# allenai/embodied-clip

Measured on AMD Instinct MI355X. Metric: env-frames/sec (CLIP encode + policy fwd/bwd + PPO update), higher is better.
Workload: dtype bf16

## Files before the change

embodied_clip_amd/_lib.py:

```python
from __future__ import annotations

import ctypes as C
import os

_HERE = os.path.dirname(os.path.abspath(__file__))
LIB_PATH = os.environ.get("EC_AMD_LIB") or os.path.join(_HERE, "lib", "libec_amd.so")

c_void_p, c_int, c_size_t, c_float = C.c_void_p, C.c_int, C.c_size_t, C.c_float

SIGNATURES = {
    "ec_version": (c_int, []),
    "ec_strerror": (C.c_char_p, [c_int]),
    "ec_bind_streams": (c_int, [c_void_p, c_int, c_int]),
    "ec_stream_pair_overlap": (c_int, [c_void_p, c_void_p, c_int, c_void_p]),
    "ec_conv_bf16": (c_int, [c_void_p] * 5 + [c_int] * 8 + [c_void_p]),
    "ec_conv_bf16_ld": (c_int, [c_void_p] * 5 + [c_int] * 9 + [c_void_p]),
    "ec_conv3x3_img_pack": (c_int, [c_void_p, c_void_p, c_int, c_void_p]),
    "ec_conv3x3_img_bf16": (c_int, [c_void_p] * 4 + [c_int] * 5 + [c_void_p]),
    "ec_conv3x3_img_bf16_ld": (c_int, [c_void_p] * 4 + [c_int] * 6 + [c_void_p]),
    "ec_bneck3_packed_elems": (c_size_t, [c_int]),
    "ec_bneck3_pack_weights": (c_int, [c_void_p] * 4 + [c_int, c_void_p]),
    "ec_bneck_conv123_bf16": (c_int, [c_void_p] * 6 + [c_int] * 4 + [c_void_p]),
    "ec_bneck_packed_elems": (c_size_t, [c_int]),
    "ec_bneck_pack_weights": (c_int, [c_void_p] * 3 + [c_int, c_void_p]),
# ... 28 lines not shown
    "ec_rn50_workspace_bytes": (c_size_t, [c_void_p, c_int]),
    "ec_rn50_out_channels": (c_int, [c_void_p]),
    "ec_rn50_out_spatial": (c_int, [c_void_p]),
    "ec_rn50_forward": (c_int, [c_void_p, c_void_p, c_int, c_void_p, c_size_t, c_void_p, c_int, c_void_p]),
    "ec_stem_conv1_depth": (c_int, [c_void_p, c_float, c_float, c_void_p, c_void_p, c_void_p] + [c_int] * 4 + [c_void_p]),
    "ec_rn50_forward_depth": (c_int, [c_void_p, c_void_p, c_float, c_float, c_void_p, c_int, c_void_p, c_size_t, c_void_p, c_int,
                                      c_void_p]),
    "ec_spatial_mean_pair_bf16": (c_int, [c_void_p] * 3 + [c_int] * 3 + [c_void_p]),
    "ec_rn50_rgbd_workspace_bytes": (c_size_t, [c_void_p, c_int]),
    "ec_rn50_embed_rgbd": (c_int, [c_void_p, c_void_p, c_int, C.POINTER(c_float), C.POINTER(c_float), c_void_p, c_float, c_float,
                                   c_void_p, c_int, c_void_p, c_size_t, c_void_p, c_int, c_void_p]),
    "ec_rn50_num_ops": (c_int, [c_void_p]),
    "ec_rn50_plan_hash": (C.c_uint64, [c_void_p]),
    "ec_rn50_set_conv8_min_tiles": (c_int, [c_void_p, c_int]),
    "ec_rn50_set_l1_rebuild": (c_int, [c_void_p, c_int]),
    "ec_text_create": (c_int, [C.POINTER(c_void_p), c_int, c_int, c_int, c_int, c_int, c_int, c_void_p, c_size_t, c_void_p,
                               c_size_t]),
    "ec_text_destroy": (None, [c_void_p]),
    "ec_text_workspace_bytes": (c_size_t, [c_void_p, c_int]),
    "ec_text_forward": (c_int, [c_void_p, c_void_p, c_int, c_void_p, c_size_t, c_void_p, c_void_p]),
    "ec_probe_head": (c_int, [c_int, c_void_p, c_void_p, c_void_p, c_int, c_int, c_int, c_void_p, c_void_p, c_void_p,
                              c_void_p, c_void_p]),
    "ec_probe_pool3": (c_int, [c_void_p, c_void_p, c_int, c_int, c_int, c_int, c_void_p]),
    "ec_conv1x1_pair_pool_bf16": (c_int, [c_void_p] * 9 + [c_int] * 6 + [c_void_p]),
    "ec_conv1x1_pair_bf16": (c_int, [c_void_p] * 11 + [C.c_long, c_int, c_int, c_int, c_void_p]),
    "ec_conv1x1_pair_rebuild_bf16": (c_int, [c_void_p] * 13 + [C.c_long, c_int, c_int, c_int, c_void_p]),
    "ec_stem_conv1_u8": (c_int, [c_void_p, C.POINTER(c_float), C.POINTER(c_float), c_void_p, c_void_p, c_void_p]
                         + [c_int] * 4 + [c_void_p]),
    "ec_rn50_forward_u8": (c_int, [c_void_p, c_void_p, C.POINTER(c_float), C.POINTER(c_float), c_int, c_void_p,
                                   c_size_t, c_void_p, c_int, c_void_p]),
    "ec_gemm_f32": (c_int, [c_void_p] * 3 + [c_int] * 3 + [C.c_long] * 4 + [c_int, c_int] + [c_void_p] * 3 + [c_int]
                    + [c_void_p] * 2 + [c_int, c_void_p]),
    "ec_policy_create": (c_int, [C.POINTER(c_void_p), c_void_p]),
    "ec_policy_destroy": (None, [c_void_p]),
    "ec_policy_num_param_tensors": (c_int, [c_void_p]),
    "ec_policy_flat_size": (c_size_t, [c_void_p]),
    "ec_policy_param_offset": (c_int, [c_void_p, c_int, C.POINTER(c_size_t), C.POINTER(c_size_t)]),
    "ec_policy_workspace_bytes": (c_size_t, [c_void_p, c_int, c_int, c_int]),
    "ec_policy_forward": (c_int, [c_void_p, c_void_p, c_void_p, c_int, c_void_p, c_void_p, c_void_p, c_int, c_int,
                                  c_void_p, c_size_t, c_int, c_void_p, c_void_p, c_void_p]),
    "ec_policy_forward2": (c_int, [c_void_p, c_void_p, c_void_p, c_void_p, c_int, c_void_p, c_void_p, c_void_p, c_int, c_int,
# ... 207 lines not shown
```

embodied_clip_amd/csrc/rn50.hip:

```cpp
#include <stdlib.h>

#include <new>
#include <vector>

#include "common.h"


namespace {

enum OpKind { OP_STEM1, OP_CONV, OP_POOL, OP_PAIR, OP_BNECK, OP_STEM7, OP_BTAIL, OP_CAT, OP_CONV_POOLOUT };

constexpr int BUF_NONE = -1, BUF_IN = -2, BUF_OUT = -3;

struct Slot { size_t w = 0, b = 0; };

struct Conv {
    int src, dst, res;
    int H, W, Cin, Cout, ks, pool, act;
    int stride;
    Slot at;
    int ldo = 0, ocol = 0;
    int img_max = 0;
    size_t wimg_off = 0;
};

// ... 17 lines not shown

}

struct ec_rn50 {
    int width, res, out_c, out_sp;
    int tv = 0;
    std::vector<Op> ops;
    size_t max_elems_per_frame;
    const float* stem_w;
    const uint16_t* w;
    const float* bias;
    size_t n_w, n_b;
    int conv8_min_tiles = 0;
    int layers4[4] = {0, 0, 0, 0};
    int l1_rebuild = 0;
    uint16_t* wbneck = nullptr;
    float* bias_cat = nullptr;
    ~ec_rn50() {
        if (wbneck) (void)hipFree(wbneck);
        if (bias_cat) (void)hipFree(bias_cat);
    }
};

namespace {
constexpr int NBUF = 5;
inline size_t align_up(size_t v, size_t a) { return (v + a - 1) / a * a; }

enum TowerKind { CLIP = 0, TV_BOTTLENECK = 1, TV_BASIC = 2 };

struct Blk {
    int li, planes, inplanes, stride;
    int R, Ro;
    int x, out;
    int y;
    bool ds, last_of_layer;
    Slot c1, c2, c3, dsc;
};
struct Arch {
    TowerKind kind; int width, R1;
    bool l1_rebuild;
    Slot stem[3], total; std::vector<Blk> B;
};

Arch walk_arch(TowerKind kind, int width, int sc, const int* layers4, int R, bool l1_rebuild = false) {
    Arch a{kind, width, R, l1_rebuild};
    Slot& at = a.total;
    auto take = [&](size_t Cout, size_t K) { const Slot s = at; at.w += Cout * K; at.b += Cout; return s; };
    a.stem[0] = take(kind == CLIP ? sc : width, 0);
    if (kind == CLIP) { a.stem[1] = take(sc, (size_t)9 * sc); a.stem[2] = take(width, (size_t)9 * sc); }
    const int expansion = kind == TV_BASIC ? 1 : 4;
    int inplanes = width, x = 0;
    for (int li = 0; li < 4; ++li)
        for (int b = 0; b < layers4[li]; ++b) {
            Blk k{li, width << li, inplanes, (b == 0 && li > 0) ? 2 : 1};
            const size_t p = k.planes, in = inplanes;
            k.ds = k.stride > 1 || inplanes != k.planes * expansion;
            k.last_of_layer = b + 1 == layers4[li];
            k.R = R; k.Ro = R / k.stride;
            k.x = x; k.y = k.out = (x == 0) ? 4 : 0;
            k.c1 = take(p, kind == TV_BASIC ? 9 * in : in);
// ... 203 lines not shown
                           : ec_bneck_pack_weights(h->w + o.c2.at.w, h->w + o.c3.at.w, h->wbneck + o.wpack_off, o.c2.Cin, nullptr);
        else if (o.kind == OP_CONV && o.c.img_max) rc = ec_conv3x3_img_pack(h->w + o.c.at.w, h->wbneck + o.c.wimg_off, o.c.Cin, nullptr);
        if (rc != EC_OK) return EC_ERR_LAUNCH;
    }
    (void)hipStreamSynchronize(nullptr);
    return EC_OK;
}

int stem_channels(int width) { return (width / 2 + 31) / 32 * 32; }

size_t plan_tower(std::vector<Op>& ops, const Arch& a, int res) {
    ops.clear();
    Plan p{ops};
    const int width = a.width, sc = stem_channels(width);
    const int x0 = a.B.empty() ? BUF_OUT : a.B[0].x;
    if (a.kind == CLIP) {
        const int R = res / 2;
        p.push(Op{OP_STEM1, mk_conv(BUF_IN, 1, BUF_NONE, res, res, 3, sc, 3, 0, EC_ACT_RELU, a.stem[0])}, R, R, sc);
        p.conv(mk_conv(1, 2, BUF_NONE, R, R, sc, sc, 3, 0, EC_ACT_RELU, a.stem[1]));
        p.conv(mk_conv(2, x0, BUF_NONE, R, R, sc, width, 3, 1, EC_ACT_RELU, a.stem[2]));
    } else {
        p.push(Op{OP_STEM7, mk_conv(BUF_IN, x0, BUF_NONE, res, res, 3, width, 7, 0, EC_ACT_RELU, a.stem[0])}, a.R1, a.R1, width);
    }
    Given g;
    for (size_t i = 0; i < a.B.size(); ++i)
        if (a.kind == TV_BASIC) plan_basic(p, a.B[i]);
        else g = plan_bottleneck(p, a, i, g);
    return p.mx;
}

bool l1_rebuild_ok(const Arch& a) {
    return a.kind == CLIP && a.B.size() >= 3 && a.B[0].ds && block_form(a, 0) == F_PAIR1 && block_form(a, 1) == F_PAIR1;
}

int rn50_build(ec_rn50_t** out, TowerKind kind, int width, const int* layers4, int input_resolution, const void* stem_w,
               const void* w_bf16, size_t n_w, const float* bias, size_t n_bias) {
    if (!out || !layers4 || !stem_w || !w_bf16 || !bias) return EC_ERR_ARG;
    if (width % 32 != 0 || width < 32 || input_resolution % 32 != 0) return EC_ERR_SHAPE;
    if (kind == TV_BASIC && (input_resolution < 32 || layers4[0] < 1 || layers4[1] < 1 || layers4[2] < 1 || layers4[3] < 1)) return EC_ERR_SHAPE;
    const int res = input_resolution;
    const Arch a = walk_arch(kind, width, stem_channels(width), layers4, res / 4);
    if (n_w != a.total.w || n_bias != a.total.b) return EC_ERR_SHAPE;
    ec_rn50* h = new (std::nothrow) ec_rn50();
    if (!h) return EC_ERR_ALLOC;
    h->width = width; h->res = res; h->tv = kind;
    std::copy(layers4, layers4 + 4, h->layers4);
    h->stem_w = (const float*)stem_w; h->w = (const uint16_t*)w_bf16; h->bias = bias;
// ... 25 lines not shown

extern "C" void ec_rn50_destroy(ec_rn50_t* h) { delete h; }
extern "C" int ec_rn50_out_channels(const ec_rn50_t* h) { return h ? h->out_c : 0; }
extern "C" int ec_rn50_out_spatial(const ec_rn50_t* h) { return h ? h->out_sp : 0; }
extern "C" int ec_rn50_num_ops(const ec_rn50_t* h) { return h ? (int)h->ops.size() : 0; }

extern "C" uint64_t ec_rn50_plan_hash(const ec_rn50_t* h) {
    if (!h) return 0;
    uint64_t x = 1469598103934665603ull;
    auto mix = [&](long v) {
        for (int i = 0; i < 8; ++i) { x ^= (uint64_t)((v >> (8 * i)) & 0xff); x *= 1099511628211ull; }
    };
    mix(ec_version()); mix((long)ec_config_hash());
    mix(h->width); mix(h->res); mix(h->conv8_min_tiles); mix(h->tv);
    if (h->l1_rebuild) mix(h->l1_rebuild);
    for (const Op& o : h->ops) {
        const Conv& c = o.kind == OP_PAIR || o.kind == OP_BNECK ? o.c3 : o.kind == OP_BTAIL ? o.c2 : o.c;
        long f[24] = {o.kind, c.src, c.dst, c.res, c.H, c.W, c.Cin, c.Cout, c.ks, c.pool, c.act, c.stride, -1, -1, 0, -1, 0, c.ldo, c.ocol, 0, -1, 0, 0, 0};
        if (o.kind == OP_POOL) {
            const long p[12] = {OP_POOL, o.pl.src, o.pl.dst, -1, o.pl.H, o.pl.W, o.pl.C, o.pl.C, 0, 0, 0, 1};
            std::copy(p, p + 12, f);
            f[17] = o.pl.ldo; f[18] = o.pl.ocol; f[23] = o.pl.pool_of;
        }
        if (o.kind == OP_PAIR) { f[12] = o.fold_ds ? o.ds.src : -1; f[13] = o.next_c1.dst; f[14] = o.next_c1.Cout; f[15] = o.pooled_dst; }
        if (o.kind == OP_BNECK) { f[1] = o.c2.src; f[8] = 3; f[16] = o.fold_c1; }
        if (o.kind == OP_BTAIL) { f[3] = -1; f[6] = o.cat.Ka + o.cat.Kb; f[12] = o.ds.src; f[14] = o.cat.Ka; f[19] = 1; }
        if (o.kind == OP_CAT) { f[0] = OP_CONV; f[14] = o.cat.Ka; f[19] = 1; }
        if (o.kind == OP_CONV_POOLOUT) { f[0] = OP_CONV; f[20] = o.pd.dst; f[21] = o.pd.ld; f[22] = o.pd.col; }
        for (long v : f) mix(v);
    }
    return x;
}

extern "C" int ec_rn50_set_conv8_min_tiles(ec_rn50_t* h, int n) {
    if (!h) return EC_ERR_ARG;
    h->conv8_min_tiles = n > 0 ? n : 0;
    return EC_OK;
}

extern "C" int ec_rn50_set_l1_rebuild(ec_rn50_t* h, int on) {
    if (!h) return EC_ERR_ARG;
    const Arch a = walk_arch((TowerKind)h->tv, h->width, stem_channels(h->width), h->layers4, h->res / 4, on != 0);
    if (!l1_rebuild_ok(a)) return EC_ERR_UNSUPPORTED;
    if ((on != 0) == (h->l1_rebuild != 0)) return EC_OK;
    std::vector<Op> ops;
    const size_t mx = plan_tower(ops, a, h->res);
    size_t tot = 0, btot = 0;
    plan_offsets(ops, tot, btot);
    if (mx != h->max_elems_per_frame) return EC_ERR_UNSUPPORTED;
    h->ops.swap(ops);
    h->l1_rebuild = on != 0;
    return EC_OK;
}

extern "C" size_t ec_rn50_workspace_bytes(const ec_rn50_t* h, int batch) {
    if (!h || batch <= 0) return 0;
    return NBUF * align_up(h->max_elems_per_frame * 2 * (size_t)batch, 256);
}

namespace {
struct FrameIn {
    enum Kind { F32, U8, DEPTH, RGBD } kind;
    const void* p;
    const float *mean3, *std3;
    float scale, shift;
    const float* stem_w9;
    const float* depth = nullptr;
// ... 77 lines not shown
        return ec_conv1x1_pair_rebuild_bf16(r.buf(c3.src), h->w + c3.at.w, h->bias + c3.at.b, r.buf(o.id_c3.src), h->w + o.id_c3.at.w,
                                            h->bias + o.id_c3.at.b, r.buf(o.id_ds.src), h->w + o.id_ds.at.w, h->bias + o.id_ds.at.b,
                                            r.buf(c3.dst), h->w + c1.at.w, h->bias + c1.at.b, r.buf(c1.dst), (long)r.nb * c3.H * c3.W,
                                            c3.Cin, c3.Cout, c1.Cout, r.stream);
    int rc = ec_conv1x1_pair_bf16(r.buf(c3.src), h->w + c3.at.w, h->bias + c3.at.b, o.fold_ds ? r.buf(o.ds.src) : nullptr,
                                  o.fold_ds ? h->w + o.ds.at.w : nullptr, o.fold_ds ? h->bias + o.ds.at.b : nullptr, r.opt(c3.res),
                                  o.no_y ? nullptr : r.buf(c3.dst), h->w + c1.at.w, h->bias + c1.at.b, r.buf(c1.dst), (long)r.nb * c3.H * c3.W, c3.Cin, c3.Cout,
                                  c1.Cout, r.stream);
    if (rc == EC_ERR_SHAPE && !o.fold_ds) {
        rc = run_conv(r, c3);
        if (rc == EC_OK) rc = run_conv(r, c1);
    }
    return rc;
}

bool bneck_fused(int nb) { return nb >= ec_config().rn50_bneck; }

int run_bneck(const Run& r, const Op& o) {
    const ec_rn50* h = r.h;
    const Conv &c1 = o.c1, &c2 = o.c2, &c3 = o.c3;
    if (bneck_fused(r.nb) && o.fold_c1)
        return ec_bneck_conv123_bf16(r.buf(c3.res), h->wbneck + o.wpack_off, h->bias + c1.at.b, h->bias + c2.at.b, h->bias + c3.at.b,
                                     r.buf(c3.dst), r.nb, c3.H, c3.W, c2.Cin, r.stream);
    if (bneck_fused(r.nb))
        return ec_bneck_conv23_bf16(r.buf(c2.src), h->wbneck + o.wpack_off, h->bias + c2.at.b, h->bias + c3.at.b, r.buf(c3.res),
                                    r.buf(c3.dst), r.nb, c3.H, c3.W, c2.Cin, r.stream);
    int rc = o.fold_c1 ? run_conv(r, c1) : EC_OK;
    if (rc == EC_OK) rc = run_conv(r, c2);
    return rc == EC_OK ? run_conv(r, c3) : rc;
}
// ... 30 lines not shown
    const size_t frame_bytes = (size_t)h->res * h->res * (in.kind == FrameIn::DEPTH ? 1 : 3) * (in.u8() ? 1 : 4);
    const size_t out_stride = (size_t)h->out_sp * h->out_sp * h->out_c;
    const hipStream_t stream = (hipStream_t)stream_main;
    auto pass = [&](Run r) -> int {
        for (const Op& o : h->ops) {
            int rc;
            switch (o.kind) {
                case OP_STEM1:
                case OP_STEM7: rc = run_stem(r, o); break;
                case OP_POOL: rc = run_pool(r, o); break;
                case OP_PAIR: rc = run_pair(r, o); break;
                case OP_BNECK: rc = run_bneck(r, o); break;
                case OP_BTAIL: rc = run_btail(r, o); break;
                case OP_CAT: rc = run_cat(r, o); break;
                case OP_CONV_POOLOUT: rc = run_conv_poolout(r, o); break;
                default: rc = run_conv(r, o.c);
            }
            if (rc != EC_OK) return rc;
        }
        return EC_OK;
    };
    unsigned char* const base = (unsigned char*)workspace;
    for (int b0 = 0; b0 < batch; b0 += chunk) {
        const int nb = std::min(chunk, batch - b0);
        const void* frames = (const unsigned char*)in.p + (size_t)b0 * frame_bytes;
        int rc;
        if (!rgbd) {
            const bool d = in.kind == FrameIn::DEPTH;
            rc = pass(Run{h, in, d ? nullptr : frames, d ? (const float*)frames : nullptr, nb, base, bufsz,
                          (uint16_t*)feat + (size_t)b0 * out_stride, stream, false});
// ... 52 lines not shown
```

embodied_clip_amd/encoder.py:

```python
from __future__ import annotations

import ctypes as C
from typing import Dict, List, Optional, Tuple

import torch

from . import _lib

BN_EPS = 1e-5


def _fold(w: torch.Tensor, sd: Dict[str, torch.Tensor], bn: str) -> Tuple[torch.Tensor, torch.Tensor]:
    g, b = sd[bn + ".weight"].float(), sd[bn + ".bias"].float()
    mu, var = sd[bn + ".running_mean"].float(), sd[bn + ".running_var"].float()
    s = g / torch.sqrt(var + BN_EPS)
    return w.float() * s.view(-1, 1, 1, 1), b - mu * s


def _layers(sd) -> List[int]:
    out = []
    for li in range(1, 5):
        n = 0
        while f"layer{li}.{n}.conv1.weight" in sd:
            n += 1
# ... 133 lines not shown
                self.h = None
        except Exception:
            pass

    def plan_hash(self) -> str:
        return f"{self.lib.ec_rn50_plan_hash(self.h):016x}"

    def set_conv8_min_tiles(self, n: int) -> None:
        _lib.check(self.lib.ec_rn50_set_conv8_min_tiles(self.h, int(n)), "ec_rn50_set_conv8_min_tiles")

    def set_l1_rebuild(self, on: bool = True) -> bool:
        rc = self.lib.ec_rn50_set_l1_rebuild(self.h, int(bool(on)))
        if rc == -6:
            return False
        _lib.check(rc, "ec_rn50_set_l1_rebuild")
        return True

    def _workspace(self, n: int) -> torch.Tensor:
        need = self.lib.ec_rn50_workspace_bytes(self.h, n)
        if self._ws is None or self._ws.numel() < need:
            self._ws = torch.empty(need, dtype=torch.uint8, device=self.device)
        return self._ws

    @_lib.on_device
    def forward(self, rgb: torch.Tensor, out: Optional[torch.Tensor] = None) -> torch.Tensor:
        assert rgb.is_cuda and rgb.dtype == torch.float32 and rgb.is_contiguous()
        B, R, R2, c3 = rgb.shape
        assert R == self.input_resolution and R2 == R and c3 == 3, rgb.shape
        S, Cc = self.out_spatial, self.out_channels
        if out is None:
# ... 478 lines not shown


@_guard_first
def conv1x1_pair_rebuild_bf16(a, w3, b3, i0, wi0, bi0, i1, wi1, bi1, w2, b2):
    lib = _lib.load()
    M, K0 = a.shape
    N, N2 = w3.shape[0], w2.shape[0]
    y = torch.empty((M, N), dtype=torch.bfloat16, device=a.device)
    z = torch.empty((M, N2), dtype=torch.bfloat16, device=a.device)
    _lib.check(lib.ec_conv1x1_pair_rebuild_bf16(a.data_ptr(), w3.data_ptr(), b3.data_ptr(), i0.data_ptr(), wi0.data_ptr(), bi0.data_ptr(),
                                                i1.data_ptr(), wi1.data_ptr(), bi1.data_ptr(), y.data_ptr(), w2.data_ptr(), b2.data_ptr(),
                                                z.data_ptr(), M, K0, N, N2, _lib.stream_ptr()), "ec_conv1x1_pair_rebuild_bf16")
    return y, z


def pack_text(sd: Dict[str, torch.Tensor]):
    sd = {k: v.detach().cpu().float() for k, v in sd.items()}
    vocab, D = sd["token_embedding.weight"].shape
    ctx = sd["positional_embedding"].shape[0]
    E = sd["text_projection"].shape[1]
    n = 0
    while f"transformer.resblocks.{n}.ln_1.weight" in sd:
        n += 1
    ws, fs = [], [sd["token_embedding.weight"].reshape(-1), sd["positional_embedding"].reshape(-1)]
    for i in range(n):
        p = f"transformer.resblocks.{i}."
        ws += [sd[p + "attn.in_proj_weight"], sd[p + "attn.out_proj.weight"], sd[p + "mlp.c_fc.weight"],
               sd[p + "mlp.c_proj.weight"]]
        fs += [sd[p + "ln_1.weight"], sd[p + "ln_1.bias"], sd[p + "attn.in_proj_bias"], sd[p + "attn.out_proj.bias"],
               sd[p + "ln_2.weight"], sd[p + "ln_2.bias"], sd[p + "mlp.c_fc.bias"], sd[p + "mlp.c_proj.bias"]]
# ... 63 lines not shown
```

embodied_clip_amd/engine.py:

```python
from __future__ import annotations

from collections import OrderedDict
from typing import Dict, List, Optional

import os
import random

import torch

from . import _lib
from . import synthetic as syn
from .dist import (allreduce_flat, check_job_seed, collective_active, gather_actor_counts, global_minibatch_sizes,
                   minibatch_bounds)
from .episodes import EpisodeTracker, NavEpisodeTracker, nav_env_tensors
from .encoder import AttentionPool, ClipTextEncoder, ImageNetBasicTrunk, ImageNetRN50Trunk, RN50Trunk, ViTEmbedder
from .policy import PolicyHandle
from .imitation import imitation_loss_raw, imitation_scratch
from .ppo import PPO_NARROW_MAX_A, FlatAdam, linear_decay_lr, ppo_loss_raw, ppo_wide_scratch

IMAGENET_ENCODERS = {
    "imagenet_rn18": ((2, 2, 2, 2), "basic", ImageNetBasicTrunk),
    "imagenet_rn34": ((3, 4, 6, 3), "basic", ImageNetBasicTrunk),
    "imagenet_rn50": ((3, 4, 6, 3), "bottleneck", ImageNetRN50Trunk),
}
# ... 340 lines not shown
            if frames_host:
                fshape = (n,) + tuple(self.env.frames.shape[2:])
                sl.stage = [torch.empty(fshape, dtype=self.env.frames.dtype, device=d) for _ in range(2)]
                sl.copy_stream = copy_streams[i]
                sl.copied = [torch.cuda.Event() for _ in range(2)]
                sl.consumed = [None, None]
                sl.k = 0
            self.slices.append(sl)
        self.encode_frames = n
        self._conv8_min_tiles = (50 if n >= 128 else (75 if n >= 64 else 0)) if ns == 2 else 0
        for e in encs:
            e.set_conv8_min_tiles(self._conv8_min_tiles)
        if encoder == "rn50":
            for e in encs:
                e.set_l1_rebuild(True)
        fused = os.environ.get("EC_ACT_FUSED_SAMPLE", "1") != "0"
        self._act_fused = fused and self.A + 1 <= 8
        self._act_wide = fused and 8 < self.A + 1 <= 257 and self.H <= 3576
        self.trunk_events: List = []
        self.time_trunk = False

    @property
    def feat(self) -> torch.Tensor:
        return self.slices[0].feat if self.ns == 1 else torch.cat([sl.feat for sl in self.slices], dim=1)

    @property
    def feat2(self) -> Optional[torch.Tensor]:
        if not self.dual:
            return None
        return self.slices[0].feat2 if self.ns == 1 else torch.cat([sl.feat2 for sl in self.slices], dim=1)
# ... 576 lines not shown
```

include/ec_amd.h:

```cpp
#ifndef EC_AMD_H
#define EC_AMD_H

#include <stddef.h>
#include <stdint.h>

#ifdef __cplusplus
extern "C" {
#endif

typedef void* ec_stream_t;
typedef void* ec_event_t;

enum {
    EC_OK = 0,
    EC_ERR_ARG = -1,
    EC_ERR_SHAPE = -2,
    EC_ERR_LAUNCH = -3,
    EC_ERR_WORKSPACE = -4,
    EC_ERR_ALLOC = -5,
    EC_ERR_UNSUPPORTED = -6
};

enum { EC_ACT_NONE = 0, EC_ACT_RELU = 1, EC_ACT_QUICKGELU = 2 };

// ... 41 lines not shown

int ec_stem_conv1(const float* rgb_nhwc, const float* w, const float* bias, void* out,
                  int B, int H, int W, int Cout, ec_stream_t stream);

int ec_stem_conv1_depth(const float* depth, float scale, float shift, const float* w9, const float* bias, void* out,
                        int B, int H, int W, int Cout, ec_stream_t stream);

int ec_conv1x1_pair_bf16(const void* a0, const void* w0, const float* b0, const void* a1, const void* w1,
                         const float* b1, const void* res, void* y, const void* w2, const float* b2, void* z,
                         long M, int K0, int N, int N2, ec_stream_t stream);

int ec_conv1x1_pair_rebuild_bf16(const void* a, const void* w3, const float* b3, const void* i0, const void* wi0,
                                 const float* bi0, const void* i1, const void* wi1, const float* bi1, void* y,
                                 const void* w2, const float* b2, void* z, long M, int K0, int N, int N2,
                                 ec_stream_t stream);

int ec_conv1x1_pair_pool_bf16(const void* a0, const void* w0, const float* b0, const void* res, void* y,
                              void* y_pooled, const void* w2, const float* b2, void* z, int B, int H, int W, int K0,
                              int N, int N2, ec_stream_t stream);

int ec_stem_conv1_u8(const uint8_t* rgb_u8_nhwc, const float* h_mean3, const float* h_std3, const float* w,
                     const float* bias, void* out, int B, int H, int W, int Cout, ec_stream_t stream);

size_t ec_bneck_packed_elems(int C);
int ec_bneck_pack_weights(const void* w2, const void* w3, void* packed, int C, ec_stream_t stream);
int ec_bneck_conv23_bf16(const void* c1, const void* packed, const float* b2, const float* b3,
                         const void* x, void* y, int B, int H, int W, int C, ec_stream_t stream);

size_t ec_bneck3_packed_elems(int C);
int ec_bneck3_pack_weights(const void* w1, const void* w2, const void* w3, void* packed, int C, ec_stream_t stream);
// ... 39 lines not shown
int ec_rn50_forward(const ec_rn50_t* h, const float* rgb_nhwc, int batch, void* workspace, size_t ws_bytes,
                    void* feat_bf16_nhwc, int chunk, ec_stream_t stream);
int ec_rn50_forward_u8(const ec_rn50_t* h, const uint8_t* rgb_u8_nhwc, const float* h_mean3, const float* h_std3,
                       int batch, void* workspace, size_t ws_bytes, void* feat_bf16_nhwc, int chunk,
                       ec_stream_t stream);
int ec_rn50_forward_depth(const ec_rn50_t* h, const float* depth, float scale, float shift, const float* stem_w9, int batch,
                          void* workspace, size_t ws_bytes, void* feat_bf16_nhwc, int chunk, ec_stream_t stream);
size_t ec_rn50_rgbd_workspace_bytes(const ec_rn50_t* h, int pairs);
int ec_rn50_embed_rgbd(const ec_rn50_t* h, const void* rgb, int rgb_u8, const float* h_mean3, const float* h_std3,
                       const float* depth, float scale, float shift, const float* stem_w9, int pairs, void* workspace,
                       size_t ws_bytes, float* embed, int chunk, ec_stream_t stream);
int ec_rn50_num_ops(const ec_rn50_t* h);
uint64_t ec_rn50_plan_hash(const ec_rn50_t* h);
int ec_rn50_set_conv8_min_tiles(ec_rn50_t* h, int n);
int ec_rn50_set_l1_rebuild(ec_rn50_t* h, int on);


enum {
    EC_GEMM_A_BF16 = 1,
    EC_GEMM_B_BF16 = 2,
    EC_GEMM_RELU = 4,
    EC_GEMM_ACCUMULATE = 8,
    EC_GEMM_SPLIT_PARTS = 16,
    EC_GEMM_3PRODUCTS = 32
};
int ec_gemm_f32(const void* A, const void* B, float* C, int M, int N, int K, long sam, long sak, long sbk, long sbn,
                int ldc, int flags, const float* bias, const float* gbias, const int* gidx, int group,
                const float* dmask, const float* rowscale, int splitk, ec_stream_t stream);

typedef struct {
// ... 231 lines not shown
```

Measured before the change: 63750.

## Fuse CLIP stem conv3 with avgpool and layer1 first 1x1 conv

Adds a new kernel that computes the third 3x3 stem conv with ReLU and 2x2 average pooling, then immediately applies the first bottleneck's 1x1 conv on the pooled tile while it is still in LDS. Both the pooled activation and the c1 output are written. A new plan op and setter wire it into the RN50 tower, and the engine enables it by default for rn50. The goal is to avoid one kernel launch and one round-trip through global memory for the pooled stem output. The cost is a specialized kernel tied to fixed channel counts (32 in, 64/64 out) that falls back to the old path for other shapes.

```diff
diff --git a/embodied_clip_amd/_lib.py b/embodied_clip_amd/_lib.py
--- a/embodied_clip_amd/_lib.py
+++ b/embodied_clip_amd/_lib.py
@@ -66,6 +66,7 @@
     "ec_rn50_plan_hash": (C.c_uint64, [c_void_p]),
     "ec_rn50_set_conv8_min_tiles": (c_int, [c_void_p, c_int]),
     "ec_rn50_set_l1_rebuild": (c_int, [c_void_p, c_int]),
+    "ec_rn50_set_stem_chain": (c_int, [c_void_p, c_int]),
     "ec_text_create": (c_int, [C.POINTER(c_void_p), c_int, c_int, c_int, c_int, c_int, c_int, c_void_p, c_size_t, c_void_p,
                                c_size_t]),
     "ec_text_destroy": (None, [c_void_p]),
@@ -77,6 +78,7 @@
     "ec_conv1x1_pair_pool_bf16": (c_int, [c_void_p] * 9 + [c_int] * 6 + [c_void_p]),
     "ec_conv1x1_pair_bf16": (c_int, [c_void_p] * 11 + [C.c_long, c_int, c_int, c_int, c_void_p]),
     "ec_conv1x1_pair_rebuild_bf16": (c_int, [c_void_p] * 13 + [C.c_long, c_int, c_int, c_int, c_void_p]),
+    "ec_stem3_pool_conv1_bf16": (c_int, [c_void_p] * 7 + [c_int] * 6 + [c_void_p]),
     "ec_stem_conv1_u8": (c_int, [c_void_p, C.POINTER(c_float), C.POINTER(c_float), c_void_p, c_void_p, c_void_p]
                          + [c_int] * 4 + [c_void_p]),
     "ec_rn50_forward_u8": (c_int, [c_void_p, c_void_p, C.POINTER(c_float), C.POINTER(c_float), c_int, c_void_p,
diff --git a/embodied_clip_amd/csrc/rn50.hip b/embodied_clip_amd/csrc/rn50.hip
--- a/embodied_clip_amd/csrc/rn50.hip
+++ b/embodied_clip_amd/csrc/rn50.hip
@@ -8,7 +8,7 @@
 
 namespace {
 
-enum OpKind { OP_STEM1, OP_CONV, OP_POOL, OP_PAIR, OP_BNECK, OP_STEM7, OP_BTAIL, OP_CAT, OP_CONV_POOLOUT };
+enum OpKind { OP_STEM1, OP_CONV, OP_POOL, OP_PAIR, OP_BNECK, OP_STEM7, OP_BTAIL, OP_CAT, OP_CONV_POOLOUT, OP_STEM_CHAIN };
 
 constexpr int BUF_NONE = -1, BUF_IN = -2, BUF_OUT = -3;
 
@@ -56,6 +56,7 @@
     int conv8_min_tiles = 0;
     int layers4[4] = {0, 0, 0, 0};
     int l1_rebuild = 0;
+    int stem_chain = 0;
     uint16_t* wbneck = nullptr;
     float* bias_cat = nullptr;
     ~ec_rn50() {
@@ -81,11 +82,12 @@
 struct Arch {
     TowerKind kind; int width, R1;
     bool l1_rebuild;
+    bool stem_chain;
     Slot stem[3], total; std::vector<Blk> B;
 };
 
-Arch walk_arch(TowerKind kind, int width, int sc, const int* layers4, int R, bool l1_rebuild = false) {
-    Arch a{kind, width, R, l1_rebuild};
+Arch walk_arch(TowerKind kind, int width, int sc, const int* layers4, int R, bool l1_rebuild = false, bool stem_chain = false) {
+    Arch a{kind, width, R, l1_rebuild, stem_chain};
     Slot& at = a.total;
     auto take = [&](size_t Cout, size_t K) { const Slot s = at; at.w += Cout * K; at.b += Cout; return s; };
     a.stem[0] = take(kind == CLIP ? sc : width, 0);
@@ -319,15 +321,25 @@
     Plan p{ops};
     const int width = a.width, sc = stem_channels(width);
     const int x0 = a.B.empty() ? BUF_OUT : a.B[0].x;
+    Given g;
     if (a.kind == CLIP) {
         const int R = res / 2;
         p.push(Op{OP_STEM1, mk_conv(BUF_IN, 1, BUF_NONE, res, res, 3, sc, 3, 0, EC_ACT_RELU, a.stem[0])}, R, R, sc);
         p.conv(mk_conv(1, 2, BUF_NONE, R, R, sc, sc, 3, 0, EC_ACT_RELU, a.stem[1]));
-        p.conv(mk_conv(2, x0, BUF_NONE, R, R, sc, width, 3, 1, EC_ACT_RELU, a.stem[2]));
+        const Conv c3 = mk_conv(2, x0, BUF_NONE, R, R, sc, width, 3, 1, EC_ACT_RELU, a.stem[2]);
+        if (a.stem_chain) {
+            const Blk& k = a.B[0];
+            Op o{OP_STEM_CHAIN, c3};
+            o.next_c1 = mk_conv(x0, 1, BUF_NONE, k.R, k.R, k.inplanes, k.planes, 1, 0, EC_ACT_RELU, k.c1);
+            p.track(k.R, k.R, k.planes);
+            p.push(o, R / 2, R / 2, width);
+            g.c1_buf = 1;
+        } else {
+            p.conv(c3);
+        }
     } else {
         p.push(Op{OP_STEM7, mk_conv(BUF_IN, x0, BUF_NONE, res, res, 3, width, 7, 0, EC_ACT_RELU, a.stem[0])}, a.R1, a.R1, width);
     }
-    Given g;
     for (size_t i = 0; i < a.B.size(); ++i)
         if (a.kind == TV_BASIC) plan_basic(p, a.B[i]);
         else g = plan_bottleneck(p, a, i, g);
@@ -336,6 +348,10 @@
 
 bool l1_rebuild_ok(const Arch& a) {
     return a.kind == CLIP && a.B.size() >= 3 && a.B[0].ds && block_form(a, 0) == F_PAIR1 && block_form(a, 1) == F_PAIR1;
+}
+
+bool stem_chain_ok(const Arch& a) {
+    return a.kind == CLIP && a.width == 64 && stem_channels(a.width) == 32 && !a.B.empty() && a.B[0].inplanes == 64 && a.B[0].planes == 64;
 }
 
 int rn50_build(ec_rn50_t** out, TowerKind kind, int width, const int* layers4, int input_resolution, const void* stem_w,
@@ -391,6 +407,7 @@
     mix(ec_version()); mix((long)ec_config_hash());
     mix(h->width); mix(h->res); mix(h->conv8_min_tiles); mix(h->tv);
     if (h->l1_rebuild) mix(h->l1_rebuild);
+    if (h->stem_chain) mix(0x5c00 + h->stem_chain);
     for (const Op& o : h->ops) {
         const Conv& c = o.kind == OP_PAIR || o.kind == OP_BNECK ? o.c3 : o.kind == OP_BTAIL ? o.c2 : o.c;
         long f[24] = {o.kind, c.src, c.dst, c.res, c.H, c.W, c.Cin, c.Cout, c.ks, c.pool, c.act, c.stride, -1, -1, 0, -1, 0, c.ldo, c.ocol, 0, -1, 0, 0, 0};
@@ -403,6 +420,7 @@
         if (o.kind == OP_BNECK) { f[1] = o.c2.src; f[8] = 3; f[16] = o.fold_c1; }
         if (o.kind == OP_BTAIL) { f[3] = -1; f[6] = o.cat.Ka + o.cat.Kb; f[12] = o.ds.src; f[14] = o.cat.Ka; f[19] = 1; }
         if (o.kind == OP_CAT) { f[0] = OP_CONV; f[14] = o.cat.Ka; f[19] = 1; }
+        if (o.kind == OP_STEM_CHAIN) { f[13] = o.next_c1.dst; f[14] = o.next_c1.Cout; }
         if (o.kind == OP_CONV_POOLOUT) { f[0] = OP_CONV; f[20] = o.pd.dst; f[21] = o.pd.ld; f[22] = o.pd.col; }
         for (long v : f) mix(v);
     }
@@ -415,19 +433,34 @@
     return EC_OK;
 }
 
-extern "C" int ec_rn50_set_l1_rebuild(ec_rn50_t* h, int on) {
-    if (!h) return EC_ERR_ARG;
-    const Arch a = walk_arch((TowerKind)h->tv, h->width, stem_channels(h->width), h->layers4, h->res / 4, on != 0);
-    if (!l1_rebuild_ok(a)) return EC_ERR_UNSUPPORTED;
-    if ((on != 0) == (h->l1_rebuild != 0)) return EC_OK;
+namespace {
+int replan(ec_rn50_t* h, const Arch& a, int l1_rebuild, int stem_chain) {
     std::vector<Op> ops;
     const size_t mx = plan_tower(ops, a, h->res);
     size_t tot = 0, btot = 0;
     plan_offsets(ops, tot, btot);
     if (mx != h->max_elems_per_frame) return EC_ERR_UNSUPPORTED;
     h->ops.swap(ops);
-    h->l1_rebuild = on != 0;
+    h->l1_rebuild = l1_rebuild;
+    h->stem_chain = stem_chain;
     return EC_OK;
+}
+}
+
+extern "C" int ec_rn50_set_l1_rebuild(ec_rn50_t* h, int on) {
+    if (!h) return EC_ERR_ARG;
+    const Arch a = walk_arch((TowerKind)h->tv, h->width, stem_channels(h->width), h->layers4, h->res / 4, on != 0, h->stem_chain != 0);
+    if (!l1_rebuild_ok(a)) return EC_ERR_UNSUPPORTED;
+    if ((on != 0) == (h->l1_rebuild != 0)) return EC_OK;
+    return replan(h, a, on != 0, h->stem_chain);
+}
+
+extern "C" int ec_rn50_set_stem_chain(ec_rn50_t* h, int on) {
+    if (!h) return EC_ERR_ARG;
+    const Arch a = walk_arch((TowerKind)h->tv, h->width, stem_channels(h->width), h->layers4, h->res / 4, h->l1_rebuild != 0, on != 0);
+    if (!stem_chain_ok(a)) return EC_ERR_UNSUPPORTED;
+    if ((on != 0) == (h->stem_chain != 0)) return EC_OK;
+    return replan(h, a, h->l1_rebuild, on != 0);
 }
 
 extern "C" size_t ec_rn50_workspace_bytes(const ec_rn50_t* h, int batch) {
@@ -535,6 +568,18 @@
     return rc;
 }
 
+int run_stem_chain(const Run& r, const Op& o) {
+    const ec_rn50* h = r.h;
+    const Conv &c3 = o.c, &c1 = o.next_c1;
+    int rc = ec_stem3_pool_conv1_bf16(r.buf(c3.src), h->w + c3.at.w, h->bias + c3.at.b, r.buf(c3.dst), h->w + c1.at.w, h->bias + c1.at.b,
+                                      r.buf(c1.dst), r.nb, c3.H, c3.W, c3.Cin, c3.Cout, c1.Cout, r.stream);
+    if (rc == EC_ERR_SHAPE) {
+        rc = run_conv(r, c3);
+        if (rc == EC_OK) rc = run_conv(r, c1);
+    }
+    return rc;
+}
+
 bool bneck_fused(int nb) { return nb >= ec_config().rn50_bneck; }
 
 int run_bneck(const Run& r, const Op& o) {
@@ -595,6 +640,7 @@
                 case OP_BTAIL: rc = run_btail(r, o); break;
                 case OP_CAT: rc = run_cat(r, o); break;
                 case OP_CONV_POOLOUT: rc = run_conv_poolout(r, o); break;
+                case OP_STEM_CHAIN: rc = run_stem_chain(r, o); break;
                 default: rc = run_conv(r, o.c);
             }
             if (rc != EC_OK) return rc;
diff --git a/embodied_clip_amd/csrc/stem3_chain.hip b/embodied_clip_amd/csrc/stem3_chain.hip
--- /dev/null
+++ b/embodied_clip_amd/csrc/stem3_chain.hip
@@ -0,0 +1,315 @@
+#include <stdlib.h>
+
+#include <type_traits>
+#include <utility>
+
+#include "common.h"
+
+namespace {
+
+typedef unsigned int u32x4 __attribute__((ext_vector_type(4)));
+
+struct ChainArgs {
+    const uint16_t *in, *w3, *w1;
+    const float *b3, *b1;
+    uint16_t *x, *c1;
+    int H, W, ntiles;
+    unsigned in_bytes;
+};
+
+constexpr int CIN = 32, COUT = 64, N2 = 64;
+constexpr int KSTEPS = 9 * CIN / 16, CB = CIN / 16, FN = COUT / 32, K3 = 9 * CIN;
+constexpr int K1STEPS = COUT / 16, FN1 = N2 / 32;
+constexpr int TR = 8, TC = 16, RT = TR / 2;
+constexpr int CPP = CIN / 8;
+constexpr int PITCH = CIN * 2 + 16;
+constexpr int RW = TC + 2, NR = TR + 2, RPB = RW * PITCH;
+constexpr int REGION = NR * RPB;
+constexpr int NCH = NR * RW * CPP;
+constexpr int IT = (NCH + 63) / 64;
+constexpr int W3_BYTES = KSTEPS * COUT * 32, W1_BYTES = K1STEPS * N2 * 32;
+constexpr int OP = COUT * 2 + 16;
+constexpr int FIXED = W3_BYTES + W1_BYTES + (COUT + N2) * 4;
+static_assert(REGION % 16 == 0, "image alignment");
+static_assert(2 * 32 * OP <= REGION, "both staging images fit the footprint region");
+static_assert(W3_BYTES + W1_BYTES < 65536, "ds_read immediates are 16 bits");
+static_assert(COUT == N2, "one staging pitch");
+
+__device__ __forceinline__ float dppq_xor1(float v) {
+    return __builtin_bit_cast(float, __builtin_amdgcn_update_dpp(0, __builtin_bit_cast(int, v), 0xB1, 0xF, 0xF, true));
+}
+__device__ __forceinline__ float dppq_xor2(float v) {
+    return __builtin_bit_cast(float, __builtin_amdgcn_update_dpp(0, __builtin_bit_cast(int, v), 0x4E, 0xF, 0xF, true));
+}
+__device__ __forceinline__ float relu1(float x) {
+    const int b = __builtin_bit_cast(int, x);
+    return __builtin_bit_cast(float, b > 0 ? b : 0);
+}
+__device__ __forceinline__ int wunit(int n, int hh) { return ((2 * n + hh) ^ ((n >> 3) & 1)) << 4; }
+
+template <int R>
+struct FragRing { u32x4 f[R]; };
+
+template <int NW, int LEADK>
+__global__ __launch_bounds__(NW * 64, 1) void stem3_chain_kernel(ChainArgs p) {
+    constexpr int G = RT + FN;
+    constexpr int RING = (LEADK + 1) * G;
+    static_assert(G * LEADK <= 15, "lgkmcnt is a 4-bit counter");
+    extern __shared__ __attribute__((aligned(16))) unsigned char sm[];
+    float* sB3 = reinterpret_cast<float*>(sm + W3_BYTES + W1_BYTES);
+    float* sB1 = sB3 + COUT;
+    const int tid = threadIdx.x, lane = tid & 63, wave = tid >> 6;
+    unsigned char* img = sm + FIXED + wave * REGION;
+    const int px = lane & 31, h = lane >> 5;
+
+    ec_stage_all<COUT * (K3 / 8), NW * 64, u32x4>(
+        tid,
+        [&](int idx) { return *reinterpret_cast<const u32x4*>(p.w3 + (long)(idx / (K3 / 8)) * K3 + (idx % (K3 / 8)) * 8); },
+        [&](int idx, const u32x4& v) {
+            const int n = idx / (K3 / 8), c = idx % (K3 / 8);
+            *reinterpret_cast<u32x4*>(sm + (c >> 1) * (COUT * 32) + wunit(n, c & 1)) = v;
+        });
+    ec_stage_all<N2 * (COUT / 8), NW * 64, u32x4>(
+        tid,
+        [&](int idx) { return *reinterpret_cast<const u32x4*>(p.w1 + (long)(idx / (COUT / 8)) * COUT + (idx % (COUT / 8)) * 8); },
+        [&](int idx, const u32x4& v) {
+            const int n = idx / (COUT / 8), c = idx % (COUT / 8);
+            *reinterpret_cast<u32x4*>(sm + W3_BYTES + (c >> 1) * (N2 * 32) + wunit(n, c & 1)) = v;
+        });
+    for (int i = tid; i < COUT; i += NW * 64) sB3[i] = p.b3[i];
+    for (int i = tid; i < N2; i += NW * 64) sB1[i] = p.b1[i];
+    __syncthreads();
+
+    const int GW = gridDim.x * NW;
+    const int lb = (int)ec_xcd_remap(blockIdx.x, gridDim.x);
+    const int nseg = p.W / TC, nrow = p.H / TR;
+    const int Hp = p.H >> 1, Wp = p.W >> 1;
+
+    constexpr int TAIL = IT - NR;
+    static_assert(RW - 16 == 2 && TAIL == 2 && NCH == NR * 64 + NR * 8, "pass geometry");
+    const unsigned rowb = (unsigned)p.W * (CIN * 2);
+    constexpr unsigned OOB = 0xFFFFF000u;
+    const unsigned lane16 = (unsigned)lane * 16u;
+    const unsigned l_oob = lane < CPP ? OOB : 0u;
+    const unsigned t_go = (unsigned)(lane >> 3) * rowb + 16u * (CIN * 2) + (unsigned)(lane & 7) * 16u;
+    const unsigned t_edge = ((lane >> 3) == 0 ? 1u : 0u) | ((lane >> 3) == 1 ? 2u : 0u) | ((lane & 4) ? 8u : 0u);
+    unsigned char* const f_lds = img + (lane / CPP) * PITCH + (lane % CPP) * 16;
+    unsigned char* const t_lds = img + (lane >> 3) * RPB + (16 + ((lane >> 2) & 1)) * PITCH + (lane & 3) * 16;
+#if defined(__HIP_DEVICE_COMPILE__)
+    const __amdgpu_buffer_rsrc_t rs_in = __builtin_amdgcn_make_buffer_rsrc((void*)p.in, 0, p.in_bytes, 0x00020000);
+#endif
+    const int wc = (0x76452310u >> (4 * (px >> 2))) & 7, dy = (px >> 1) & 1, dx = px & 1;
+    const unsigned a_lds = (unsigned)(unsigned long)(__attribute__((address_space(3))) unsigned char*)img +
+                           (unsigned)(dy * RPB + (2 * wc + dx) * PITCH + h * 16);
+    const unsigned w_lds = (unsigned)(unsigned long)(__attribute__((address_space(3))) unsigned char*)sm + (unsigned)wunit(px, h);
+
+    u32x4 nxt[IT];
+    struct Coord { int sg, rr, b; };
+    auto decode = [&](int t_) {
+        const int t = __builtin_amdgcn_readfirstlane(t_);
+        return Coord{t % nseg, (t / nseg) % nrow, t / (nseg * nrow)};
+    };
+    const Coord step = decode(GW);
+    auto advance = [&](Coord c) {
+        c.sg += step.sg; c.rr += step.rr; c.b += step.b;
+        if (c.sg >= nseg) { c.sg -= nseg; ++c.rr; }
+        if (c.rr >= nrow) { c.rr -= nrow; ++c.b; }
+        return c;
+    };
+    auto fetch = [&](Coord c) {
+        const int sgi = __builtin_amdgcn_readfirstlane(c.sg), rr = __builtin_amdgcn_readfirstlane(c.rr);
+        const int b = __builtin_amdgcn_readfirstlane(c.b);
+        const int y0 = TR * rr - 1, x0 = TC * sgi - 1;
+        const unsigned base = (unsigned)((((long)b * p.H + y0) * p.W + x0) * (CIN * 2));
+        const bool top = y0 < 0, bottom = y0 + NR - 1 >= p.H, left = x0 < 0, right = x0 + RW - 1 >= p.W;
+        const unsigned tm0 = (top ? 1u : 0u) | (right ? 8u : 0u), tm1 = (bottom ? 2u : 0u) | (right ? 8u : 0u);
+        const unsigned lbad = left ? l_oob : 0u;
+#if defined(__HIP_DEVICE_COMPILE__)
+        [&]<int... I>(std::integer_sequence<int, I...>) {
+            (([&] {
+                 unsigned off;
+                 if constexpr (I < NR) {
+                     const unsigned srow = ((I == 0 && top) || (I == NR - 1 && bottom)) ? OOB : base + (unsigned)I * rowb;
+                     off = ((unsigned)__builtin_amdgcn_readfirstlane((int)srow) + lane16) | lbad;
+                 } else if constexpr (I == NR) {
+                     off = (base + t_go) | ((t_edge & tm0) ? OOB : 0u);
+                 } else {
+                     off = ((unsigned)__builtin_amdgcn_readfirstlane((int)(base + 8u * rowb)) + t_go) | ((t_edge & tm1) ? OOB : 0u);
+                 }
+                 nxt[I] = __builtin_amdgcn_raw_buffer_load_b128(rs_in, (int)off, 0, 0);
+             }()),
+             ...);
+        }(std::make_integer_sequence<int, IT>{});
+#endif
+    };
+
+    auto land = [&] {
+        [&]<int... I>(std::integer_sequence<int, I...>) {
+            (([&] {
+                 if constexpr (I < NR) *reinterpret_cast<u32x4*>(f_lds + I * RPB) = nxt[I];
+                 else if (I == NR || lane < 16) *reinterpret_cast<u32x4*>(t_lds + (I - NR) * 8 * RPB) = nxt[I];
+             }()),
+             ...);
+        }(std::make_integer_sequence<int, IT>{});
+    };
+
+    int t = __builtin_amdgcn_readfirstlane(lb * NW + wave);
+    if (t >= p.ntiles) return;
+    Coord cc = decode(t), cn = cc;
+    fetch(cc);
+    land();
+    t += GW;
+    bool more = t < p.ntiles;
+    if (more) { cn = advance(cn); fetch(cn); }
+    for (;;) {
+        f32x16_t acc[RT][FN];
+#pragma unroll
+        for (int n = 0; n < FN; ++n)
+#pragma unroll
+            for (int g = 0; g < 4; ++g) {
+                const float4 bv = *reinterpret_cast<const float4*>(sB3 + 32 * n + 8 * g + 4 * h);
+                acc[0][n][4 * g + 0] = bv.x; acc[0][n][4 * g + 1] = bv.y; acc[0][n][4 * g + 2] = bv.z; acc[0][n][4 * g + 3] = bv.w;
+            }
+#pragma unroll
+        for (int n = 0; n < FN; ++n) asm volatile("" : "+v"(acc[0][n]) : : "memory");
+
+        FragRing<RING> ring;
+        auto issue = [&](auto sc, auto qc) {
+            constexpr int S = decltype(sc)::value, q = decltype(qc)::value;
+            constexpr int tap = S / CB, cb = S % CB, ky = tap / 3, kx = tap % 3;
+            constexpr int slot = (S % (LEADK + 1)) * G + q;
+            const unsigned al = a_lds, wl = w_lds;
+            auto& rg = ring;
+            if constexpr (q < RT) {
+                asm volatile("ds_read_b128 %0, %1 offset:%2" : "=v"(rg.f[slot]) : "v"(al), "n"((2 * q + ky) * RPB + kx * PITCH + cb * 32));
+            } else {
+                asm volatile("ds_read_b128 %0, %1 offset:%2" : "=v"(rg.f[slot]) : "v"(wl), "n"(S * (COUT * 32) + (q - RT) * 1024));
+            }
+        };
+        auto issue_step = [&](auto sc) {
+            [&]<int... Q>(std::integer_sequence<int, Q...>) { (issue(sc, std::integral_constant<int, Q>{}), ...); }
+            (std::make_integer_sequence<int, G>{});
+        };
+        [&]<int... S>(std::integer_sequence<int, S...>) { (issue_step(std::integral_constant<int, S>{}), ...); }
+        (std::make_integer_sequence<int, LEADK>{});
+        [&]<int... S>(std::integer_sequence<int, S...>) {
+            (([&] {
+                 if constexpr (S + LEADK < KSTEPS) issue_step(std::integral_constant<int, S + LEADK>{});
+                 constexpr int ahead = (S + LEADK < KSTEPS ? LEADK : KSTEPS - 1 - S) * G;
+                 asm volatile("s_waitcnt lgkmcnt(%0)" : : "n"(ahead));
+                 constexpr int base = (S % (LEADK + 1)) * G;
+#pragma unroll
+                 for (int q = 0; q < G; ++q) asm volatile("" : "+v"(ring.f[base + q]));
+#pragma unroll
+                 for (int i = RT - 1; i >= 0; --i)
+#pragma unroll
+                     for (int n = 0; n < FN; ++n)
+                         acc[i][n] = __builtin_amdgcn_mfma_f32_32x32x16_bf16(__builtin_bit_cast(bf16x8_t, ring.f[base + RT + n]),
+                                                                            __builtin_bit_cast(bf16x8_t, ring.f[base + i]),
+                                                                            S == 0 ? acc[0][n] : acc[i][n], 0, 0, 0);
+             }()),
+             ...);
+        }(std::make_integer_sequence<int, KSTEPS>{});
+
+        unsigned char* stg = img;
+        unsigned char* const pst = stg + wc * OP + h * 8;
+#pragma unroll
+        for (int i = 0; i < RT; ++i)
+#pragma unroll
+            for (int n = 0; n < FN; ++n) {
+                uint2 o[4];
+#pragma unroll
+                for (int g = 0; g < 4; ++g) {
+                    float v0 = relu1(acc[i][n][4 * g + 0]), v1 = relu1(acc[i][n][4 * g + 1]);
+                    float v2 = relu1(acc[i][n][4 * g + 2]), v3 = relu1(acc[i][n][4 * g + 3]);
+                    v0 += dppq_xor1(v0); v1 += dppq_xor1(v1); v2 += dppq_xor1(v2); v3 += dppq_xor1(v3);
+                    v0 += dppq_xor2(v0); v1 += dppq_xor2(v1); v2 += dppq_xor2(v2); v3 += dppq_xor2(v3);
+                    o[g].x = ec_pack2(0.25f * v0, 0.25f * v1);
+                    o[g].y = ec_pack2(0.25f * v2, 0.25f * v3);
+                }
+                if ((lane & 3) == 0) {
+#pragma unroll
+                    for (int g = 0; g < 4; ++g) *reinterpret_cast<uint2*>(pst + i * 8 * OP + (32 * n + 8 * g) * 2) = o[g];
+                }
+            }
+        const int sgi = __builtin_amdgcn_readfirstlane(cc.sg), rr = __builtin_amdgcn_readfirstlane(cc.rr);
+        const int b = __builtin_amdgcn_readfirstlane(cc.b);
+        constexpr int ZC = COUT / 8;
+        const long opix0 = ((long)b * Hp + RT * rr) * Wp + (TC / 2) * sgi;
+        unsigned char* const xo = reinterpret_cast<unsigned char*>(p.x + opix0 * COUT);
+        unsigned char* const co = reinterpret_cast<unsigned char*>(p.c1 + opix0 * N2);
+        const unsigned char* const srd = stg + (lane / ZC) * OP + (lane % ZC) * 16;
+        u32x4 xs[RT], cs[RT];
+#pragma unroll
+        for (int i = 0; i < RT; ++i) xs[i] = *reinterpret_cast<const u32x4*>(srd + i * 8 * OP);
+
+        f32x16_t acc1[FN1];
+#pragma unroll
+        for (int n = 0; n < FN1; ++n)
+#pragma unroll
+            for (int r = 0; r < 16; ++r) acc1[n][r] = 0.f;
+#pragma unroll
+        for (int ks = 0; ks < K1STEPS; ++ks) {
+            const s16x8_t av = *reinterpret_cast<const s16x8_t*>(stg + px * OP + ks * 32 + h * 16);
+#pragma unroll
+            for (int n = 0; n < FN1; ++n) {
+                const s16x8_t wf = *reinterpret_cast<const s16x8_t*>(sm + W3_BYTES + ks * (N2 * 32) + wunit(32 * n + px, h));
+                acc1[n] = __builtin_amdgcn_mfma_f32_32x32x16_bf16(__builtin_bit_cast(bf16x8_t, wf), __builtin_bit_cast(bf16x8_t, av), acc1[n], 0, 0, 0);
+            }
+        }
+        unsigned char* stg1 = img + 32 * OP;
+#pragma unroll
+        for (int n = 0; n < FN1; ++n)
+#pragma unroll
+            for (int g = 0; g < 4; ++g) {
+                const int lc = 32 * n + 8 * g + 4 * h;
+                const float4 bv = *reinterpret_cast<const float4*>(sB1 + lc);
+                uint2 o;
+                o.x = ec_pack2(relu1(acc1[n][4 * g + 0] + bv.x), relu1(acc1[n][4 * g + 1] + bv.y));
+                o.y = ec_pack2(relu1(acc1[n][4 * g + 2] + bv.z), relu1(acc1[n][4 * g + 3] + bv.w));
+                *reinterpret_cast<uint2*>(stg1 + px * OP + lc * 2) = o;
+            }
+#pragma unroll
+        for (int i = 0; i < RT; ++i) cs[i] = *reinterpret_cast<const u32x4*>(srd + 32 * OP + i * 8 * OP);
+        if (more) land();
+        asm volatile("" ::: "memory");
+#pragma unroll
+        for (int i = 0; i < RT; ++i) {
+            *reinterpret_cast<u32x4*>(xo + (long)i * Wp * (COUT * 2) + lane16) = xs[i];
+            *reinterpret_cast<u32x4*>(co + (long)i * Wp * (N2 * 2) + lane16) = cs[i];
+        }
+        if (!more) break;
+        cc = cn;
+        t += GW;
+        more = t < p.ntiles;
+        if (more) { cn = advance(cn); fetch(cn); }
+    }
+}
+
+template <int NW, int LEADK>
+int launch_chain(const ChainArgs& p, hipStream_t s) {
+    constexpr size_t lds = (size_t)FIXED + (size_t)NW * REGION;
+    static_assert(lds <= 160 * 1024, "LDS budget");
+    auto kern = stem3_chain_kernel<NW, LEADK>;
+    static std::atomic<uint64_t> attr_done{0};
+    if (auto attr_g_ = ec_attr_needed(attr_done)) {
+        (void)hipFuncSetAttribute(reinterpret_cast<const void*>(kern), hipFuncAttributeMaxDynamicSharedMemorySize, (int)lds);
+    }
+    const int wgs = (p.ntiles + NW - 1) / NW < 256 ? (p.ntiles + NW - 1) / NW : 256;
+    hipLaunchKernelGGL(kern, dim3((unsigned)wgs), dim3(NW * 64), lds, s, p);
+    EC_CHECK_LAUNCH();
+    return EC_OK;
+}
+
+}
+
+extern "C" int ec_stem3_pool_conv1_bf16(const void* in, const void* w3, const float* b3, void* x_out, const void* w1, const float* b1,
+                                        void* c1_out, int B, int H, int W, int Cin, int Cout, int N2_, ec_stream_t stream) {
+    if (!in || !w3 || !b3 || !x_out || !w1 || !b1 || !c1_out) return EC_ERR_ARG;
+    if (B <= 0 || H <= 0 || W <= 0 || (H % TR) != 0 || (W % TC) != 0 || Cin != CIN || Cout != COUT || N2_ != N2) return EC_ERR_SHAPE;
+    const long nt = (long)B * (H / TR) * (W / TC), bytes = (long)B * H * W * CIN * 2;
+    if (nt > 0x7fffffffL || bytes >= (1L << 32) - 4096) return EC_ERR_SHAPE;
+    ChainArgs p{(const uint16_t*)in, (const uint16_t*)w3, (const uint16_t*)w1, b3, b1, (uint16_t*)x_out, (uint16_t*)c1_out, H, W, (int)nt,
+                (unsigned)bytes};
+    return launch_chain<7, 1>(p, (hipStream_t)stream);
+}
diff --git a/embodied_clip_amd/encoder.py b/embodied_clip_amd/encoder.py
--- a/embodied_clip_amd/encoder.py
+++ b/embodied_clip_amd/encoder.py
@@ -171,6 +171,13 @@
         if rc == -6:
             return False
         _lib.check(rc, "ec_rn50_set_l1_rebuild")
+        return True
+
+    def set_stem_chain(self, on: bool = True) -> bool:
+        rc = self.lib.ec_rn50_set_stem_chain(self.h, int(bool(on)))
+        if rc == -6:
+            return False
+        _lib.check(rc, "ec_rn50_set_stem_chain")
         return True
 
     def _workspace(self, n: int) -> torch.Tensor:
@@ -679,6 +686,18 @@
     return y, z
 
 
+@_guard_first
+def stem3_pool_conv1_bf16(x, w3, b3, w1, b1):
+    lib = _lib.load()
+    B, H, W, Cin = x.shape
+    Cout, N2 = w3.shape[0], w1.shape[0]
+    xo = torch.empty((B, H // 2, W // 2, Cout), dtype=torch.bfloat16, device=x.device)
+    c1 = torch.empty((B, H // 2, W // 2, N2), dtype=torch.bfloat16, device=x.device)
+    _lib.check(lib.ec_stem3_pool_conv1_bf16(x.data_ptr(), w3.data_ptr(), b3.data_ptr(), xo.data_ptr(), w1.data_ptr(), b1.data_ptr(),
+                                            c1.data_ptr(), B, H, W, Cin, Cout, N2, _lib.stream_ptr()), "ec_stem3_pool_conv1_bf16")
+    return xo, c1
+
+
 def pack_text(sd: Dict[str, torch.Tensor]):
     sd = {k: v.detach().cpu().float() for k, v in sd.items()}
     vocab, D = sd["token_embedding.weight"].shape
diff --git a/embodied_clip_amd/engine.py b/embodied_clip_amd/engine.py
--- a/embodied_clip_amd/engine.py
+++ b/embodied_clip_amd/engine.py
@@ -378,6 +378,7 @@
         if encoder == "rn50":
             for e in encs:
                 e.set_l1_rebuild(True)
+                e.set_stem_chain(True)
         fused = os.environ.get("EC_ACT_FUSED_SAMPLE", "1") != "0"
         self._act_fused = fused and self.A + 1 <= 8
         self._act_wide = fused and 8 < self.A + 1 <= 257 and self.H <= 3576
diff --git a/include/ec_amd.h b/include/ec_amd.h
--- a/include/ec_amd.h
+++ b/include/ec_amd.h
@@ -79,6 +79,9 @@
                                  const float* bi0, const void* i1, const void* wi1, const float* bi1, void* y,
                                  const void* w2, const float* b2, void* z, long M, int K0, int N, int N2,
                                  ec_stream_t stream);
+
+int ec_stem3_pool_conv1_bf16(const void* in, const void* w3, const float* b3, void* x_out, const void* w1, const float* b1,
+                             void* c1_out, int B, int H, int W, int Cin, int Cout, int N2, ec_stream_t stream);
 
 int ec_conv1x1_pair_pool_bf16(const void* a0, const void* w0, const float* b0, const void* res, void* y,
                               void* y_pooled, const void* w2, const float* b2, void* z, int B, int H, int W, int K0,
@@ -148,6 +151,7 @@
 uint64_t ec_rn50_plan_hash(const ec_rn50_t* h);
 int ec_rn50_set_conv8_min_tiles(ec_rn50_t* h, int n);
 int ec_rn50_set_l1_rebuild(ec_rn50_t* h, int on);
+int ec_rn50_set_stem_chain(ec_rn50_t* h, int on);
 
 
 enum {
```

After: 64220, median of 6. No clear change (+0.7%).
